# Magicyw/Quadruped-PyMPC-TAMOLS

Hardware: AMD Instinct MI355X
Metric: SRBD rollouts/sec + p50 MPC-step ms at N=10k H=12; 1/2/4/8 GPU (higher is better)
Workload: dtype f32; 1 GPU; go2_trot_flat_mppi_n10000_h12_zo; num_samples=10000, rows_per_gpu=10000, horizon=12, method=mppi, parametrization=zero_order, robot=go2, gait=trot, parallelism=single GPU

## Files before the change

### quadruped-pympc-tamols_amd/csrc/srbd_device.h

```cpp
#pragma once

#include <utility>

#include "srbd_jaxrng.h"
#include "srbd_launch.h"

namespace srbd {

#ifdef SRBD_ROLLOUT_STAMPS
constexpr int RSTAMP_N = 6, RSTAMP_BLOCKS = 8192;
__device__ uint64_t g_rstamp[RSTAMP_BLOCKS * RSTAMP_N];
#define SRBD_RSTAMP(i)                                                                  \
    do {                                                                                \
        if (threadIdx.x == 0 && blockIdx.x < RSTAMP_BLOCKS) {                           \
            asm volatile("s_waitcnt vmcnt(0) lgkmcnt(0)" ::: "memory");                 \
            g_rstamp[blockIdx.x * RSTAMP_N + (i)] = __builtin_amdgcn_s_memrealtime(); \
        }                                                                               \
    } while (0)
__device__ uint64_t g_lstamp[RSTAMP_BLOCKS * 8];
__device__ uint64_t g_fstamp[64];
#define SRBD_LSTAMP(i)                                                                            \
    do {                                                                                          \
        if (threadIdx.x == 0 && blockIdx.x < RSTAMP_BLOCKS)                                       \
            g_lstamp[blockIdx.x * 8 + (i)] = __builtin_amdgcn_s_memrealtime();                    \
// ... 182 lines not shown
    const size_t ldn = (size_t)mc.ldn;
    int j = first / n, k = first - j * n;
    const int sj = stride / n, sk = stride - sj * n;
    while (j < P) {
        const int r = mc.row0 + k;
        const float v = r > 0 ? jax_noise_value(mc, k0, k1, r, j, part) : 0.0f;
        __hip_atomic_store(&job.noise[(size_t)j * ldn + k], v, __ATOMIC_RELAXED, __HIP_MEMORY_SCOPE_AGENT);
        k += sk;
        j += sj;
        if (k >= n) {
            k -= n;
            ++j;
        }
    }
}

__device__ __forceinline__ void advance_key(const ModelConst& mc, StepInput* in, int inc) {
    const uint64_t cc = (((uint64_t)in->ctr_hi << 32) | in->ctr_lo) + (uint64_t)inc;
    in->ctr_lo = (uint32_t)cc;
    in->ctr_hi = (uint32_t)(cc >> 32);
    if (mc.rng != RNG_PHILOX) {
        const uint64_t key = jax_next_key(((uint64_t)in->seed_hi << 32) | in->seed_lo, mc.rng == RNG_JAX, inc);
        in->seed_lo = (uint32_t)key;
        in->seed_hi = (uint32_t)(key >> 32);
    }
}

__device__ __forceinline__ void rng_items(const ModelConst& mc, const StepInput* __restrict__ in, const RngJob& job,
                                          int first, int stride) {
    uint64_t seed = job.seed, ctr = job.ctr;
    if (job.dev_ctr) {
        seed = ((uint64_t)in->seed_hi << 32) | in->seed_lo;
        ctr = (((uint64_t)in->ctr_hi << 32) | in->ctr_lo) + (uint64_t)job.ctr_offset;
        if (mc.rng != RNG_PHILOX) seed = jax_next_key(seed, mc.rng == RNG_JAX, job.ctr_offset);
    }
    if (mc.rng != RNG_PHILOX) return jax_rng_items(mc, seed, job, first, stride);
    const int n = mc.n_local, nq = mc.P / 4;
    int q = first / n, k = first - q * n;
    const int sq = stride / n, sk = stride - sq * n;
    while (q < nq) {
        rng_item(mc, in->sigma, (uint32_t)seed, (uint32_t)(seed >> 32), (uint32_t)ctr, (uint32_t)(ctr >> 32), k, q,
                 job.noise);
        k += sk;
        q += sq;
        if (k >= n) {
            k -= n;
            ++q;
        }
    }
}

__host__ __device__ constexpr int chunk_index(int n, int H, int S) { return (n * S) / H; }

template <int N>
struct IntC {
    static constexpr int value = N;
};
template <class F, int... Ns>
__device__ __forceinline__ void unroll_seq(F&& f, std::integer_sequence<int, Ns...>) {
    (f(IntC<Ns>{}), ...);
}

__device__ __forceinline__ void st_rec(float* p, float v) {
    __hip_atomic_store(reinterpret_cast<uint32_t*>(p), __float_as_uint(v), __ATOMIC_RELAXED, __HIP_MEMORY_SCOPE_AGENT);
}
__device__ __forceinline__ float ld_rec(const float* p) {
    return __uint_as_float(
        __hip_atomic_load(reinterpret_cast<const uint32_t*>(p), __ATOMIC_RELAXED, __HIP_MEMORY_SCOPE_AGENT));
}
template <int U>
__device__ __forceinline__ void stage_recs16(const float* __restrict__ src, float* dst, int n) {
    const int tid = threadIdx.x, T = blockDim.x, n4 = n >> 2;
    const auto rs = __builtin_amdgcn_make_buffer_rsrc((void*)src, (short)0, n * 4, 0x00020000);
    float4* d4 = reinterpret_cast<float4*>(dst);
    for (int i0 = 0; i0 < n4; i0 += U * T) {
        float4 v[U];
#pragma unroll
        for (int u = 0; u < U; ++u) {
            const auto x = __builtin_amdgcn_raw_buffer_load_b128(rs, 16 * (i0 + u * T + tid), 0, 16);
            v[u] = make_float4(__uint_as_float(x[0]), __uint_as_float(x[1]), __uint_as_float(x[2]),
                               __uint_as_float(x[3]));
        }
#pragma unroll
        for (int u = 0; u < U; ++u) {
            const int i = i0 + u * T + tid;
            if (i < n4) d4[i] = v[u];
        }
    }
}
template <int U>
__device__ __forceinline__ void stage_recs(const float* __restrict__ src, float* dst, int n) {
    const int tid = threadIdx.x, T = blockDim.x, n2 = n >> 1;
    const uint64_t* s2 = reinterpret_cast<const uint64_t*>(src);
    uint64_t* d2 = reinterpret_cast<uint64_t*>(dst);
    for (int i0 = 0; i0 < n2; i0 += U * T) {
        uint64_t v[U];
#pragma unroll
        for (int u = 0; u < U; ++u) {
            const int i = i0 + u * T + tid;
            v[u] = i < n2 ? __hip_atomic_load(s2 + i, __ATOMIC_RELAXED, __HIP_MEMORY_SCOPE_AGENT) : 0ull;
        }
#pragma unroll
        for (int u = 0; u < U; ++u) {
            const int i = i0 + u * T + tid;
            if (i < n2) d2[i] = v[u];
        }
    }
}


__device__ __forceinline__ void fold_node_lds(const ModelConst& mc, const float* st, int rec_stride, int nb, float* G) {
    __shared__ float sc_sh[TREE_FAN];
    __shared__ float gh_sh[2];
    __shared__ uint64_t gk_sh[MAXK + 1];
    const int tid = threadIdx.x, T = blockDim.x;
    const int P = mc.P, K = mc.K;
    const bool rs = mc.method == SRBD_RANDOM_SAMPLING;
    if (tid < 64) {
        const float* R = st + (size_t)tid * rec_stride;
        const bool have = tid < nb;
        const float m = have ? R[0] : 0.0f;
        const uint32_t row = have ? __float_as_uint(R[2]) : 0u;
        const uint64_t key = have ? ((uint64_t)__float_as_uint(m) << 32) | row : KEY_NONE;
        const uint64_t gk = wave_min_u64(key);
        const float beta = __uint_as_float((uint32_t)(gk >> 32));
        if (key == gk) gh_sh[1] = R[3];
        if (tid == 0) {
            gh_sh[0] = beta;
            gk_sh[MAXK] = gk;
        }
        if (have) sc_sh[tid] = rs ? 1.0f : expf(-1.0f * (m - beta));
        if (tid == 0) gk_sh[0] = gk;
    }
    __syncthreads();
    SRBD_LSTAMP(4);
    if (!rs) {
        for (int j = tid; j <= P; j += T) {
            const int off = j < P ? REC_HDR + j : 1;
            float a = 0.0f;
            int cb = 0;
            for (; cb + 8 <= nb; cb += 8) {
                float x[8];
#pragma unroll
                for (int u = 0; u < 8; ++u) x[u] = st[(size_t)(cb + u) * rec_stride + off];
#pragma unroll
                for (int u = 0; u < 8; ++u) a = a + sc_sh[cb + u] * x[u];
            }
            for (; cb < nb; ++cb) a = a + sc_sh[cb] * st[(size_t)cb * rec_stride + off];
            st_rec(&G[off], a);
        }
    }
    SRBD_LSTAMP(5);
    if (tid == 0) {
        st_rec(&G[0], gh_sh[0]);
        if (rs) st_rec(&G[1], 1.0f);
        st_rec(&G[2], __uint_as_float((uint32_t)gk_sh[MAXK]));
        st_rec(&G[3], gh_sh[1]);
    }
    if (tid < K) {
        const uint64_t kk = gk_sh[tid];
        st_rec(&G[REC_HDR + P + 2 * tid], __uint_as_float((uint32_t)kk));
        st_rec(&G[REC_HDR + P + 2 * tid + 1], __uint_as_float((uint32_t)(kk >> 32)));
    }
}

__device__ __forceinline__ bool level1_fold(const ModelConst& mc, const float* __restrict__ recs, int rec_stride,
                                            const GroupArgs& grp, int nroll, int lpb, float* st) {
    __shared__ int last_sh;
    const int tid = threadIdx.x;
    const int bpg = TREE_FAN / lpb;
    const int g = (int)blockIdx.x / bpg;
    const int nblk = min(bpg, nroll - g * bpg);
    const int nb = min(TREE_FAN, mc.nleaf - g * TREE_FAN);
    SRBD_LSTAMP(0);
    asm volatile("s_waitcnt vmcnt(0)" ::: "memory");
    __syncthreads();
    SRBD_LSTAMP(1);
    if (tid == 0) {
        const uint32_t old = __hip_atomic_fetch_add(grp.cnt + g, 1u, __ATOMIC_RELAXED, __HIP_MEMORY_SCOPE_AGENT);
        last_sh = old == (uint32_t)(nblk - 1);
    }
    __syncthreads();
    if (!last_sh) return false;
    SRBD_LSTAMP(2);
    if (tid == 0) __hip_atomic_store(grp.cnt + g, 0u, __ATOMIC_RELAXED, __HIP_MEMORY_SCOPE_AGENT);
    stage_recs16<5>(recs + (size_t)g * TREE_FAN * rec_stride, st, nb * rec_stride);
    __syncthreads();
    SRBD_LSTAMP(3);
    fold_node_lds(mc, st, rec_stride, nb, grp.grecs + (size_t)g * rec_stride);
    return true;
}

template <int CTRL, int ROWMASK>
__device__ __forceinline__ float dpp_f32(float v) {
    return __int_as_float(__builtin_amdgcn_update_dpp(0, __float_as_int(v), CTRL, ROWMASK, 0xF, false));
}
template <int LEVELS>
__device__ __forceinline__ float lane_tree_f32(float v) {
    v = v + dpp_f32<0x111, 0xF>(v);
    v = v + dpp_f32<0x112, 0xF>(v);
    v = v + dpp_f32<0x114, 0xF>(v);
    v = v + dpp_f32<0x118, 0xF>(v);
    if constexpr (LEVELS >= 5) v = v + dpp_f32<0x142, 0xA>(v);
    if constexpr (LEVELS >= 6) v = v + dpp_f32<0x143, 0xC>(v);
    return v;
}
__device__ __forceinline__ float wave_sum_f32(float v) { return lane_tree_f32<6>(v); }

constexpr int REGEN_QUADS = 16;
template <int SPL, int RG>
__device__ __forceinline__ void leaf_wsum_lanes(const ModelConst& mc, const StepInput* __restrict__ in,
                                                const float* __restrict__ base, bool zs, const float* e_sh,
                                                float* rbuf, int rec_stride, int k0, int gen = 0) {
    constexpr int CB = SPL == 4 ? 8 : 12;
    constexpr int LPL = 64 / SPL;
    const int lane = threadIdx.x & 63, w = threadIdx.x >> 6, NW = blockDim.x >> 6;
    const int P = mc.P;
    const size_t ldn = (size_t)mc.ldn;
    float e[SPL];
#pragma unroll
    for (int u = 0; u < SPL; ++u) e[u] = e_sh[SPL * lane + u];
    float* rec = rbuf + (lane / LPL) * rec_stride;
    const bool writer = (lane % LPL) == LPL - 1;
    int jreg = 0;
    if constexpr (RG && SPL == 4) {
        if (RG == 2 || (mc.method == SRBD_MPPI && mc.rng == RNG_PHILOX && in->noise_scaled == 0 && 4 * REGEN_QUADS <= P)) {
            const uint32_t key0 = in->seed_lo, key1 = in->seed_hi, c2 = in->ctr_lo, c3 = in->ctr_hi;
            const int nq = RG == 2 ? gen - 1 : REGEN_QUADS;
            for (int q = w; q < nq; q += NW) {
                float zq[4][SPL];
#pragma unroll
                for (int u = 0; u < SPL; ++u) {
                    const int k = k0 + SPL * lane + u, r = mc.row0 + k;
                    uint32_t c[4] = {(uint32_t)(r - 1), (uint32_t)q, c2, c3};
                    philox4x32_10(c, key0, key1);
                    float v[4];
                    box_muller(c[0], c[1], v[0], v[1]);
                    box_muller(c[2], c[3], v[2], v[3]);
                    const bool live = r > 0 && k < mc.n_local;
#pragma unroll
                    for (int i = 0; i < 4; ++i) zq[i][u] = live ? mc.sigma_mppi * v[i] : 0.0f;
                }
#pragma unroll
                for (int i = 0; i < 4; ++i) {
                    float p[SPL];
#pragma unroll
                    for (int u = 0; u < SPL; ++u) p[u] = e[u] * (zq[i][u] * 1.0f);
                    float a = (p[0] + p[1]) + (p[2] + p[3]);
                    a = lane_tree_f32<4>(a);
                    if (writer) rec[REC_HDR + 4 * q + i] = a;
                }
            }
            jreg = 4 * nq;
        }
    }
    for (int j0 = jreg + w; j0 <= P; j0 += CB * NW) {
        float z[CB][SPL];
#pragma unroll
        for (int b = 0; b < CB; ++b) {
            const int j = j0 + b * NW;
            const float* col = base + (size_t)(j < P ? j : 0) * ldn + SPL * lane;
            if constexpr (SPL == 4) {
                const float4 v = *reinterpret_cast<const float4*>(col);
                z[b][0] = v.x, z[b][1] = v.y, z[b][2] = v.z, z[b][3] = v.w;
            } else {
                const float2 v = *reinterpret_cast<const float2*>(col);
                z[b][0] = v.x, z[b][1] = v.y;
            }
        }
#pragma unroll
        for (int b = 0; b < CB; ++b) {
            const int j = j0 + b * NW;
            if (j > P) break;
            float p[SPL];
            if (j < P) {
                const float sj = zs ? in->sigma[j] : 1.0f;
#pragma unroll
                for (int u = 0; u < SPL; ++u) p[u] = e[u] * (z[b][u] * sj);
            } else {
#pragma unroll
                for (int u = 0; u < SPL; ++u) p[u] = e[u];
            }
            float a;
            if constexpr (SPL == 4)
                a = (p[0] + p[1]) + (p[2] + p[3]);
            else
                a = p[0] + p[1];
            a = lane_tree_f32<SPL == 4 ? 4 : 5>(a);
            if (writer) rec[j < P ? REC_HDR + j : 1] = a;
        }
    }
}

template <bool ZS>
__device__ __forceinline__ void leaf_wsum_cols(const ModelConst& mc, const StepInput* __restrict__ in,
                                               const float* __restrict__ base, const float* zst, int zstride, bool zs,
                                               const float* e_sh, float* __restrict__ rec) {
    const int tid = threadIdx.x, T = blockDim.x, P = mc.P;
    const size_t ldn = (size_t)mc.ldn;
    if ((tid >> 6) == (T >> 6) - 1) {
        const float t = wave_sum_f32(e_sh[tid & 63]);
        if ((tid & 63) == 63) st_rec(&rec[1], t);
    }
    for (int j = tid; j < P; j += T) {
        const float sj = zs ? in->sigma[j] : 1.0f;
        float first = 0.0f, tot = 0.0f;
#pragma nounroll
        for (int h = 0; h < 2; ++h) {
            float lv[16];
            if constexpr (ZS) {
#pragma unroll
                for (int i = 0; i < 16; ++i) {
                    const int r = 32 * h + 2 * i;
                    lv[i] = e_sh[r] * (zst[r * zstride + j] * sj) + e_sh[r + 1] * (zst[(r + 1) * zstride + j] * sj);
                }
            } else {
                const float4* row = reinterpret_cast<const float4*>(base + (size_t)j * ldn) + 8 * h;
                float4 v[8];
#pragma unroll
                for (int i = 0; i < 8; ++i) v[i] = row[i];
#pragma unroll
                for (int i = 0; i < 8; ++i) {
                    const int r = 32 * h + 4 * i;
                    lv[2 * i] = e_sh[r] * (v[i].x * sj) + e_sh[r + 1] * (v[i].y * sj);
                    lv[2 * i + 1] = e_sh[r + 2] * (v[i].z * sj) + e_sh[r + 3] * (v[i].w * sj);
                }
            }
#pragma unroll
            for (int n = 8; n >= 1; n >>= 1)
#pragma unroll
                for (int i = 0; i < n; ++i) lv[i] = lv[2 * i] + lv[2 * i + 1];
            if (h == 0)
                first = lv[0];
            else
                tot = first + lv[0];
        }
        st_rec(&rec[REC_HDR + j], tot);
    }
}

template <bool CEMT, bool ZS = false, bool TF = false, int RG = 0>
__device__ __forceinline__ bool block_epilogue(const ModelConst& mc, const StepInput* __restrict__ in, const int SPB,
                                               int sib, bool valid, float cost, const float* __restrict__ noise,
                                               float* __restrict__ recs, int rec_stride, float tag,
                                               const GroupArgs& grp, int nroll, float* zst = nullptr,
                                               int zstride = 0) {
    __shared__ uint64_t ks[ZS ? 64 : 256];
    __shared__ float e_sh[ZS ? 64 : 256];
    __shared__ uint64_t lmin[4];
    __shared__ uint64_t lel[CEMT ? 4 : 1][CEMT ? MAXK : 1];
    __shared__ float rbuf[TF ? 4 * ((REC_HDR + MAXP + 2 * MAXK + 3) & ~3) : 1];
    const int tid = threadIdx.x, lane = tid & 63, w = tid >> 6;
    const int lpb = SPB >> 6;
    const int P = mc.P, K = mc.K;
    const int k0 = blockIdx.x * SPB;
    const bool rs = mc.method == SRBD_RANDOM_SAMPLING;
    const uint64_t key = (sib >= 0 && valid) ? cost_key(cost, (uint32_t)(mc.row0 + k0 + sib)) : KEY_NONE;
    if (sib >= 0) ks[sib] = key;
    __syncthreads();
    constexpr bool ONE = ZS && !CEMT;
    uint64_t m1 = KEY_NONE;
    if constexpr (ONE) {
        m1 = wave_min_u64(ks[lane]);
    } else if (w < lpb) {
        const uint64_t m = wave_min_u64(ks[64 * w + lane]);
        if (lane == 0) lmin[w] = m;
    }
    if constexpr (CEMT) {
        if (K > 1) {
            for (int i = tid; i < lpb * MAXK; i += (int)blockDim.x) lel[i / MAXK][i % MAXK] = KEY_NONE;
            __syncthreads();
            const int lps = (int)blockDim.x / SPB, part = tid & (lps - 1), s = tid / lps, b = s >> 6;
            const uint64_t mine = ks[s];
            const int span = 64 / lps, i0 = 64 * b + part * span;
            int cnt = 0;
            for (int i = 0; i < span; ++i) cnt += ks[i0 + i] < mine ? 1 : 0;
            if (lps >= 2) cnt += __builtin_amdgcn_mov_dpp(cnt, 0xB1, 0xF, 0xF, true);
            if (lps == 4) cnt += __builtin_amdgcn_mov_dpp(cnt, 0x4E, 0xF, 0xF, true);
            if (part == 0 && cnt < K) lel[b][cnt] = mine;
        }
    }
    if constexpr (!ONE) __syncthreads();
    SRBD_RSTAMP(3);
    if (!rs) {
        const uint64_t lm = ONE ? m1 : (sib >= 0 ? lmin[sib >> 6] : KEY_NONE);
        if (sib >= 0) e_sh[sib] = valid ? expf(-1.0f * (cost - u2f((uint32_t)(lm >> 32)))) : 0.0f;
        __syncthreads();
        const bool zs = CEMT && zs_scaled(mc, in);
        if (SPB == 64)
            leaf_wsum_cols<ZS>(mc, in, noise + k0, zst, zstride, zs, e_sh, recs + (size_t)blockIdx.x * rec_stride);
        else if constexpr (TF) {
            if (SPB == 128)
                leaf_wsum_lanes<2, RG>(mc, in, noise + k0, zs, e_sh, rbuf, rec_stride, k0);
            else
                leaf_wsum_lanes<4, RG>(mc, in, noise + k0, zs, e_sh, rbuf, rec_stride, k0, grp.gen);
        }
    }
    SRBD_RSTAMP(4);
    const bool via_lds = TF && SPB > 64;
    float* const grec = recs + (size_t)blockIdx.x * lpb * rec_stride;
    auto put = [&](int b, int off, float v) {
        if (via_lds)
            rbuf[b * rec_stride + off] = v;
        else
            st_rec(&grec[(size_t)b * rec_stride + off], v);
    };
    auto leafmin = [&](int b) { return ONE ? m1 : lmin[b]; };
    if (tid < lpb) {
        const uint64_t m = leafmin(tid);
        put(tid, 0, u2f((uint32_t)(m >> 32)));
        put(tid, 2, u2f((uint32_t)m));
        if (rs) put(tid, 1, 1.0f);
    }
    if (sib >= 0 && key == leafmin(sib >> 6)) put(sib >> 6, 3, tag);
    for (int i = tid; i < lpb * K; i += (int)blockDim.x) {
        const int b = i / K, q = i % K;
        uint64_t kk = leafmin(b);
        if constexpr (CEMT) kk = K > 1 ? lel[b][q] : kk;
        put(b, REC_HDR + P + 2 * q, u2f((uint32_t)kk));
        put(b, REC_HDR + P + 2 * q + 1, u2f((uint32_t)(kk >> 32)));
    }
    if (via_lds) {
        __syncthreads();
        for (int i = tid; i < lpb * rec_stride; i += (int)blockDim.x) st_rec(&grec[i], rbuf[i]);
    }
    if constexpr (!CEMT) {
        if (grp.gsize > 1) {
            if (grp.fast) return true;
            if constexpr (ZS) {
                return level1_fold(mc, recs, rec_stride, grp, nroll, lpb, zst);
            } else {
                __shared__ __attribute__((aligned(16))) float st[GROUP_LDS_FLOATS];
                return level1_fold(mc, recs, rec_stride, grp, nroll, lpb, st);
            }
        }
    }
    return false;
}

constexpr uint32_t GA_FREQ_LANE = 0x10000u;

__device__ __forceinline__ float ga_sample_freq(const ModelConst& mc, const StepInput* __restrict__ in, int k) {
    if (in->ga_explicit) return mc.ga_freq[k];
    const uint64_t seed = ((uint64_t)in->seed_hi << 32) | in->seed_lo;
    if (mc.rng != RNG_PHILOX)
        return in->ga_freqs[jax_choice_index((uint32_t)(seed >> 32), (uint32_t)seed, (uint64_t)(mc.row0 + k),
                                             (uint64_t)mc.N, (uint32_t)in->ga_nfreq, mc.rng == RNG_JAX)];
    uint32_t c[4] = {(uint32_t)(mc.row0 + k), GA_FREQ_LANE, in->ctr_lo, in->ctr_hi};
    philox4x32_10(c, (uint32_t)seed, (uint32_t)(seed >> 32));
    const uint32_t i = (uint32_t)(((uint64_t)c[0] * (uint32_t)in->ga_nfreq) >> 32);
    return in->ga_freqs[i];
}

__device__ __forceinline__ void ga_contact_masks(const StepInput* __restrict__ in, int H, float f, uint32_t mask[4]) {
    const float inc = in->ga_dt * f;
    float t[4];
#pragma unroll
    for (int l = 0; l < 4; ++l) {
        t[l] = in->ga_timing[l];
        mask[l] = 0u;
    }
    for (int n = 0; n < H; ++n)
#pragma unroll
        for (int l = 0; l < 4; ++l) {
            t[l] = t[l] >= 1.0f ? 0.0f : t[l];
            t[l] = t[l] + inc;
            mask[l] |= (t[l] < in->ga_duty ? 1u : 0u) << n;
        }
}

}
```

### quadruped-pympc-tamols_amd/csrc/srbd_kernels.hip

```cpp
#include "srbd_device.h"

#include <cstdlib>

namespace srbd {

__global__ void __launch_bounds__(256) rng_kernel(const ModelConst mc, const StepInput* __restrict__ in,
                                                  const RngJob job) {
    if (job.gate && (*job.gate & ARM_CANCEL)) return;
    rng_items(mc, in, job, blockIdx.x * 256 + threadIdx.x, gridDim.x * 256);
}

__global__ void __launch_bounds__(256) transpose_kernel(const float* __restrict__ src, int n, int P, int ldn,
                                                        float* __restrict__ dst) {
    __shared__ float tile[32][33];
    const int bx = blockIdx.x * 32, by = blockIdx.y * 32;
    const int tx = threadIdx.x & 31, ty = threadIdx.x >> 5;
    for (int i = ty; i < 32; i += 8) {
        const int row = bx + i, col = by + tx;
        tile[i][tx] = (row < n && col < P) ? src[(size_t)row * P + col] : 0.0f;
    }
    __syncthreads();
    for (int i = ty; i < 32; i += 8) {
        const int col = by + i, row = bx + tx;
        if (col < P && row < n) dst[(size_t)col * ldn + row] = tile[tx][i];
// ... 31 lines not shown
};
__device__ __forceinline__ QuadLane quad_lane(const ModelConst& mc, int c) {
    QuadLane L;
    L.c = c;
    L.g = c == 2 ? -9.81f : 0.0f;
    L.Ir0 = sel3(c, mc.inertia[0], mc.inertia[3], mc.inertia[6]);
    L.Ir1 = sel3(c, mc.inertia[1], mc.inertia[4], mc.inertia[7]);
    L.Ir2 = sel3(c, mc.inertia[2], mc.inertia[5], mc.inertia[8]);
    L.Ii0 = sel3(c, mc.Iinv[0], mc.Iinv[3], mc.Iinv[6]);
    L.Ii1 = sel3(c, mc.Iinv[1], mc.Iinv[4], mc.Iinv[7]);
    L.Ii2 = sel3(c, mc.Iinv[2], mc.Iinv[5], mc.Iinv[8]);
    return L;
}

struct QuadRB {
    float er, R0, R1, R2, a1;
};
__device__ __forceinline__ QuadRB quad_rb_prep(const QuadLane& L, float r, float w) {
    const int c = L.c;
    float sn, cs;
    sincos_(r, &sn, &cs);
    const float sr = qp<QP_B0>(sn), cr = qp<QP_B0>(cs);
    const float sp = qp<QP_B1>(sn), cp = qp<QP_B1>(cs);
    const float sy = qp<QP_B2>(sn), cy = qp<QP_B2>(cs);
    const float w0 = qp<QP_B0>(w), w1 = qp<QP_B1>(w), w2 = qp<QP_B2>(w);
    float k1, k2;
    euler_rate_coefs(c, sr, cr, sp, cp, k1, k2);
    const float kw1 = k1 * w1;
    const float er0 = w0 + kw1;
    const float er = (c == 0 ? er0 : kw1) + k2 * w2;
    const float A = c == 1 ? sr : cr;
    const float B0 = c == 1 ? -cr : sr, B1 = c == 1 ? cr : -sr;
    const float Asp = A * sp;
    const float r0a = cp * cy, r0b = Asp * cy + B0 * sy;
    const float r1a = cp * sy, r1b = Asp * sy + B1 * cy;
    const float r2b = A * cp;
    const float R0 = c == 0 ? r0a : r0b;
    const float R1 = c == 0 ? r1a : r1b;
    const float R2 = c == 0 ? -sp : r2b;
    const float Iw = L.Ir0 * w0 + L.Ir1 * w1 + L.Ir2 * w2;
    const float wx = (-qp<QP_NEXT2>(w)) * qp<QP_NEXT>(Iw) + qp<QP_NEXT>(w) * qp<QP_NEXT2>(Iw);
    const float a1 = L.Ii0 * qp<QP_B0>(wx) + L.Ii1 * qp<QP_B1>(wx) + L.Ii2 * qp<QP_B2>(wx);
    return QuadRB{er, R0, R1, R2, a1};
}
__device__ __forceinline__ void quad_rb_apply(const ModelConst& mc, const QuadLane& L, const QuadRB& q, float temp,
                                              float temp2, float dt, float& p, float& v, float& r, float& w) {
    const float lin = mc.inv_m * temp + L.g;
    const float Rt = q.R0 * qp<QP_B0>(temp2) + q.R1 * qp<QP_B1>(temp2) + q.R2 * qp<QP_B2>(temp2);
    const float a2 = L.Ii0 * qp<QP_B0>(Rt) + L.Ii1 * qp<QP_B1>(Rt) + L.Ii2 * qp<QP_B2>(Rt);
    const float aa = -q.a1 + a2;
    const float pn = p + v * dt, vn = v + lin * dt, rn = r + q.er * dt, wn = w + aa * dt;
    p = pn;
    v = vn;
    r = rn;
    w = wn;
}
__device__ __forceinline__ void quad_rb_apply3(const ModelConst& mc, const QuadLane& L, const QuadRB& q, float temp,
                                               float t2x, float t2y, float t2z, float dt, float& p, float& v, float& r,
                                               float& w) {
    const float lin = mc.inv_m * temp + L.g;
    const float Rt = q.R0 * t2x + q.R1 * t2y + q.R2 * t2z;
    const float a2 = L.Ii0 * qp<QP_B0>(Rt) + L.Ii1 * qp<QP_B1>(Rt) + L.Ii2 * qp<QP_B2>(Rt);
    const float aa = -q.a1 + a2;
    const float pn = p + v * dt, vn = v + lin * dt, rn = r + q.er * dt, wn = w + aa * dt;
    p = pn;
    v = vn;
    r = rn;
    w = wn;
}
__device__ __forceinline__ void quad_rigid_body(const ModelConst& mc, const QuadLane& L, float temp, float temp2,
                                                float dt, float& p, float& v, float& r, float& w) {
    quad_rb_apply(mc, L, quad_rb_prep(L, r, w), temp, temp2, dt, p, v, r, w);
}

__device__ __forceinline__ float quad_cross(float vl, float fl) {
    const float vn1 = qp<QP_NEXT>(vl), vn2 = qp<QP_NEXT2>(vl);
    const float fn1 = qp<QP_NEXT>(fl), fn2 = qp<QP_NEXT2>(fl);
    return (-vn2) * fn1 + vn1 * fn2;
}

template <int NT, bool XG>
__device__ void final_merge(const ModelConst& mc, const StepInput* in, const float* noise, int rec_stride,
                            const GroupArgs& grp, float* lds);
__device__ void fast_tail(const ModelConst& mc, const StepInput* in, const float* noise, const float* recs,
                          int rec_stride, const GroupArgs& grp, int nroll, float* st);

#ifndef SRBD_QUAD_WPE
#define SRBD_QUAD_WPE 4
#endif
template <int KIND, int HT, int ST, bool CEMT, bool EXT, int FM = 0, bool KS = false, bool GEN = false>
__global__ void __launch_bounds__(512) __attribute__((amdgpu_waves_per_eu(SRBD_QUAD_WPE))) rollout_quad_kernel(
                                                           const std::conditional_t<KS, StepInputK, KsNone> ksi,
                                                           const ModelConst mc, const StepInput* __restrict__ in_dev,
                                                           const float* __restrict__ noise, float* __restrict__ costs,
                                                           float* __restrict__ recs, int rec_stride,
    const RngJob next_rng, int nroll, const GroupArgs grp) {
    const StepInput* __restrict__ in;
    if constexpr (KS) {
        (void)ksi;
        const auto ka = (const __attribute__((address_space(4))) StepInput*)__builtin_amdgcn_kernarg_segment_ptr();
        in = (const StepInput*)ka;
        if (blockIdx.x == 0) {
            const auto src = (const __attribute__((address_space(4))) uint32_t*)ka;
            uint32_t* dst = reinterpret_cast<uint32_t*>(const_cast<StepInput*>(in_dev));
            for (int i = threadIdx.x; i < (int)(sizeof(StepInputK) / 4); i += blockDim.x) dst[i] = src[i];
        }
    } else {
        in = in_dev;
    }
    if (grp.gate && (*grp.gate & ARM_CANCEL)) {
        if (FM && blockIdx.x == 0 && threadIdx.x == 0)
            __hip_atomic_store(grp.flag, grp.seq | ARM_CANCEL, __ATOMIC_RELAXED, __HIP_MEMORY_SCOPE_SYSTEM);
        return;
    }
    SRBD_RSTAMP(0);
#if SRBD_PRIO
    if ((int)blockIdx.x < nroll && nroll >= SRBD_PRIO_MIN) __builtin_amdgcn_s_setprio(SRBD_PRIO);
#endif
    if ((int)blockIdx.x >= nroll) {
        rng_items(mc, in, next_rng, ((int)blockIdx.x - nroll) * (int)blockDim.x + (int)threadIdx.x,
                  ((int)gridDim.x - nroll) * (int)blockDim.x);
        SRBD_RSTAMP(5);
        return;
    }

    constexpr bool CT = HT > 0 && (KIND == SRBD_ZERO_ORDER || ST > 0);
    const int SPB = (int)blockDim.x >> 2;
    const int H = CT ? HT : mc.H;
    const int S = CT ? ST : mc.S;
    const int PL = CT ? (KIND == SRBD_ZERO_ORDER ? 3 * HT : (KIND == SRBD_LINEAR_SPLINE ? 3 * (ST + 1) : 12 * ST))
                      : mc.PL;
    constexpr bool ZST = CT && KIND == SRBD_ZERO_ORDER && !EXT && HT <= 12;
    static_assert(!GEN || (ZST && HT % 4 == 0 && !CEMT), "GEN: the zero-order LDS-staged form, H % 4 == 0");
    constexpr int PCT = ZST ? 12 * HT : 1;
    constexpr int ZSTR = PCT + 1;
    __shared__ __attribute__((aligned(16))) float zst[ZST ? (64 * ZSTR > GROUP_LDS_FLOATS ? 64 * ZSTR : GROUP_LDS_FLOATS) : 1];
    __shared__ float bls[ZST ? PCT : 1];
    __shared__ float sls[ZST && CEMT ? PCT : 1];
    const int tid = threadIdx.x;
    const int q4 = tid & 3;
    const int c = q4 < 3 ? q4 : 2;
    const int sib = tid >> 2;
    const int k = blockIdx.x * SPB + sib;
    const bool valid = k < mc.n_local;
    const size_t ldn = (size_t)mc.ldn;
    const float* __restrict__ nz = noise + k;
    const float* __restrict__ best = in->best;
    const bool zs = CEMT && zs_scaled(mc, in);

    const QuadLane L = quad_lane(mc, c);
    const float Qp = sel3(c, mc.Q[0], mc.Q[1], mc.Q[2]), Qv = sel3(c, mc.Q[3], mc.Q[4], mc.Q[5]);
    const float Qr = sel3(c, mc.Q[6], mc.Q[7], mc.Q[8]), Qw = sel3(c, mc.Q[9], mc.Q[10], mc.Q[11]);
    const float* st = in->state;
    const float* rf = in->ref;
    const float rp = sel3(c, rf[0], rf[1], rf[2]), rv = sel3(c, rf[3], rf[4], rf[5]);
    const float rr = sel3(c, rf[6], rf[7], rf[8]), rw = sel3(c, rf[9], rf[10], rf[11]);
    float feet[4];
#pragma unroll
    for (int l = 0; l < 4; ++l) feet[l] = sel3(c, st[12 + 3 * l], st[13 + 3 * l], st[14 + 3 * l]);
    float p = sel3(c, st[0], st[1], st[2]), v = sel3(c, st[3], st[4], st[5]);
    float r = sel3(c, st[6], st[7], st[8]), w = sel3(c, st[9], st[10], st[11]);
    float cost = 0.0f;
    const float rwc = sel3(c, mc.cost_r[0], mc.cost_r[1], mc.cost_r[2]);
    float fprev[4];
    constexpr bool LEGP = !EXT;
    const int lq = q4;
    uint32_t lmask[4];
#pragma unroll
    for (int l = 0; l < 4; ++l) lmask[l] = lq == l ? ~0u : 0u;
    float footL[3];
#pragma unroll
    for (int q = 0; q < 3; ++q) footL[q] = st[12 + 3 * lq + q];
    constexpr int NCL = ZST ? HT : 1;
    float clreg[NCL];
    if constexpr (ZST) {
#pragma unroll
        for (int n = 0; n < HT; ++n) clreg[n] = in->contact[lq][n];
    }

    constexpr int NPRE = !CT ? 1 : (KIND == SRBD_ZERO_ORDER ? HT : (KIND == SRBD_LINEAR_SPLINE ? ST + 1 : 4 * ST));
    float pre[LEGP ? 3 : 4][NPRE];
    const int cblk = LEGP ? lq * PL
                          : (KIND == SRBD_ZERO_ORDER ? c * HT : (KIND == SRBD_LINEAR_SPLINE ? c * (ST + 1) : 4 * c));
    const auto nrs = __builtin_amdgcn_make_buffer_rsrc((void*)noise, (short)0, mc.P * mc.ldn * 4, 0x00020000);
    const int voff = (cblk * mc.ldn + k) * 4;
    const float* __restrict__ bl = best + cblk;
    const float* __restrict__ sl = in->sigma + cblk;
    if constexpr (ZST) {
        for (int j = tid; j < PCT; j += 256) {
            bls[j] = best[j];
            if constexpr (CEMT) sls[j] = in->sigma[j];
        }
    }
    auto load_slot = [&](const int i) __attribute__((always_inline)) {
#pragma unroll
        for (int l = 0; l < (LEGP ? 3 : 4); ++l) {
            const int jr = LEGP ? (KIND == SRBD_ZERO_ORDER ? l * HT + i
                                   : (KIND == SRBD_LINEAR_SPLINE ? l * (ST + 1) + i : 10 * (i >> 2) + 4 * l + (i & 3)))
                                : l * PL + (KIND == SRBD_CUBIC_SPLINE ? 10 * (i >> 2) + (i & 3) : i);
#ifdef SRBD_DIAG_NOLOAD
            const float nzv = (float)(voff + jr * mc.ldn) * 1e-9f;
#else
            const float nzv = __uint_as_float(__builtin_amdgcn_raw_buffer_load_b32(nrs, voff, jr * mc.ldn * 4, 0));
#endif
            if constexpr (ZST) {
                pre[l][i] = nzv;
            } else if constexpr (CEMT) {
                const float sj = sl[jr];
                pre[l][i] = bl[jr] + nzv * (zs ? sj : 1.0f);
            } else {
                pre[l][i] = bl[jr] + nzv;
            }
        }
    };
    constexpr int PW = (EXT && KIND == SRBD_ZERO_ORDER) ? (NPRE < 4 ? NPRE : 4) : NPRE;
    constexpr int CLEAD = 2;
    constexpr bool CWIN = CT && CEMT && KIND == SRBD_CUBIC_SPLINE && ST > 1;
    if constexpr (GEN) {
    } else if constexpr (CWIN) {
#pragma unroll
        for (int i = 0; i < 4; ++i) load_slot(i);
    } else if constexpr (CT) {
#pragma unroll
        for (int i = 0; i < PW; ++i) load_slot(i);
    }
    if constexpr (ZST) {
        asm volatile("s_waitcnt lgkmcnt(0)" ::: "memory");
        __builtin_amdgcn_s_barrier();
    }

    float dep = p;
    auto gen4 = [&](const int s, auto is) __attribute__((always_inline)) {
        const int r = mc.row0 + k;
        const bool live = r > 0 && valid;
        const uint32_t d = (uint32_t)(r - 1);
#pragma unroll
        for (int q = 0; q < 3; ++q) {
            uint32_t cc[4] = {d, (uint32_t)(lq * (PL / 4) + q * (HT / 4) + s), is->ctr_lo, is->ctr_hi};
            philox4x32_10(cc, is->seed_lo, is->seed_hi);
            float v[4];
            box_muller(cc[0], cc[1], v[0], v[1]);
            box_muller(cc[2], cc[3], v[2], v[3]);
#pragma unroll
            for (int i = 0; i < 4; ++i) pre[q][(4 * s + i) % NPRE] = live ? mc.sigma_mppi * v[i] : 0.0f;
        }
    };
    auto step = [&](const int n, auto EX) __attribute__((always_inline)) {
        if constexpr (GEN)
            if (n % 4 == 0) gen4(n / 4, step_ptr(in, cost));
        if constexpr (CT && PW < NPRE)
            if (n + PW < NPRE) load_slot(n + PW);
        if constexpr (CWIN) {
#pragma unroll
            for (int q = 1; q < (CWIN ? ST : 1); ++q) {
                const int at = q * HT / ST - CLEAD;
                if (n == (at > 0 ? at : 0))
#pragma unroll
                    for (int i = 4 * q; i < 4 * q + 4; ++i) load_slot(i);
            }
        }
        const auto is = step_ptr(in, dep);
        float cl[4] = {0.0f, 0.0f, 0.0f, 0.0f};
        if constexpr (!ZST)
#pragma unroll
            for (int l = 0; l < 4; ++l) cl[l] = is->contact[l][n];
        const float fref = is->fzref[n];
        const float dt = mc.dts[n];
        const float sq = mc.sq[n], somq = mc.somq[n], sa = mc.sa[n], sb = mc.sb[n], scc = mc.sc[n], sd = mc.sd[n];
        const int idx = CT && KIND != SRBD_ZERO_ORDER ? chunk_index(n, HT, ST) : mc.sidx[n];
        float temp, temp2, ex = 0.0f;
        if constexpr (LEGP) {
            const float clq = ZST ? clreg[ZST ? n : 0]
                                  : __uint_as_float((__float_as_uint(cl[0]) & lmask[0]) | (__float_as_uint(cl[1]) & lmask[1]) |
                                                    (__float_as_uint(cl[2]) & lmask[2]) | (__float_as_uint(cl[3]) & lmask[3]));
            const int lbase = lq * PL;
            auto PQ = [&](int q, int i, int j) {
                if constexpr (ZST) {
                    if constexpr (CEMT) return bls[lbase + j] + pre[q][i] * (zs ? sls[lbase + j] : 1.0f);
                    return bls[lbase + j] + pre[q][i];
                } else if constexpr (CT) {
                    return pre[q][i];
                } else {
                    const float z = nz[(size_t)(lbase + j) * ldn];
                    return best[lbase + j] + (zs ? z * in->sigma[lbase + j] : z);
                }
            };
            float rq[3];
#pragma unroll
            for (int q = 0; q < 3; ++q) {
                if (KIND == SRBD_ZERO_ORDER) {
                    rq[q] = PQ(q, n, n + q * H);
                } else if (KIND == SRBD_LINEAR_SPLINE) {
                    const int o = idx + q * (S + 1);
                    rq[q] = somq * PQ(q, idx, o) + sq * PQ(q, idx + 1, o + 1);
                } else {
                    const int o = 10 * idx + 4 * q;
                    const float p0 = PQ(q, 4 * idx, o), p1 = PQ(q, 4 * idx + 1, o + 1), p2 = PQ(q, 4 * idx + 2, o + 2),
                                p3 = PQ(q, 4 * idx + 3, o + 3);
                    const float phi = 0.5f * ((p2 - p1) + (p1 - p0));
                    const float phin = 0.5f * ((p3 - p2) + (p2 - p1));
                    rq[q] = sa * p1 + sb * phi + scc * p2 + sd * phin;
                }
            }
            const float fz = clamp_cs((fref + rq[2]) * clq, mc.grf_min, mc.grf_max);
            const float lo = mc.neg_mu * fz, hi = mc.mu * fz;
            const float fx = clamp_cs(third(rq[0] * clq), lo, hi), fy = clamp_cs(third(rq[1] * clq), lo, hi);
            const float vx = footL[0] - qp<QP_B0>(p), vy = footL[1] - qp<QP_B1>(p), vz = footL[2] - qp<QP_B2>(p);
            float sm[6] = {fx * clq, fy * clq, fz * clq, ((-vz) * fy + vy * fz) * clq, (vz * fx + (-vx) * fz) * clq,
                           ((-vy) * fx + vx * fy) * clq};
#pragma unroll
            for (int i = 0; i < 6; ++i) {
                sm[i] = sm[i] + qp<QP_XOR1>(sm[i]);
                sm[i] = sm[i] + qp<QP_XOR2>(sm[i]);
            }
            temp = sel3(c, sm[0], sm[1], sm[2]);
            temp2 = sel3(c, sm[3], sm[4], sm[5]);
            dep = sm[5];
            quad_rb_apply3(mc, L, quad_rb_prep(L, r, w), temp, sm[3], sm[4], sm[5], dt, p, v, r, w);
        } else {
        float tf[4], tt[4];
#pragma unroll
        for (int l = 0; l < 4; ++l) {
            const int base = l * PL;
            auto P = [&](int i, int j) {
                if constexpr (CT) {
                    return pre[l][i];
                } else {
                    const float z = nz[(size_t)(base + j) * ldn];
                    return best[base + j] + (zs ? z * in->sigma[base + j] : z);
                }
            };
            float raw;
            if (KIND == SRBD_ZERO_ORDER) {
                raw = P(n, n + c * H);
            } else if (KIND == SRBD_LINEAR_SPLINE) {
                const int o = idx + c * (S + 1);
                raw = somq * P(idx, o) + sq * P(idx + 1, o + 1);
            } else {
                const int o = 10 * idx + 4 * c;
                const float p0 = P(4 * idx, o), p1 = P(4 * idx + 1, o + 1), p2 = P(4 * idx + 2, o + 2),
                            p3 = P(4 * idx + 3, o + 3);
                const float phi = 0.5f * ((p2 - p1) + (p1 - p0));
                const float phin = 0.5f * ((p3 - p2) + (p2 - p1));
                raw = sa * p1 + sb * phi + scc * p2 + sd * phin;
            }
            float zp = clamp_cs((fref + raw) * cl[l], mc.grf_min, mc.grf_max);
            const float xy = third(raw * cl[l]);
            const float fz = qp<QP_B2>(c == 2 ? zp : xy);
            const float f = c == 2 ? fz : clamp_cs(xy, mc.neg_mu * fz, mc.mu * fz);
            tf[l] = f * cl[l];
            tt[l] = quad_cross(feet[l] - p, f) * cl[l];
            if constexpr (decltype(EX)::value) {
                const float u = c == 2 ? f - (cl[l] != 0.0f ? fref : 0.0f) : f;
                float term = (u * rwc) * u;
                if (n > 0) {
                    const float d = f - fprev[l];
                    term = term + (d * mc.cost_smooth) * d;
                }
                {
                    float vv = fabsf(xy) - mc.mu * fz;
                    vv = vv > 0.0f ? vv : 0.0f;
                    const float cone = (vv * mc.cost_cone) * vv;
                    term = c < 2 ? term + cone : term;
                }
                ex = ex + term;
                fprev[l] = f;
            }
        }
        temp = (tf[0] + tf[1]) + (tf[2] + tf[3]);
        temp2 = (tt[0] + tt[1]) + (tt[2] + tt[3]);
        dep = temp2;
        quad_rigid_body(mc, L, temp, temp2, dt, p, v, r, w);
        }
        const float ep = p - rp, ev = v - rv, er_ = r - rr, ew = w - rw;
        const float tp = (ep * Qp) * ep, tv = (ev * Qv) * ev, tr = (er_ * Qr) * er_, tw = (ew * Qw) * ew;
        cost = cost + (((tp + tv) + tr) + tw);
        if constexpr (decltype(EX)::value) {
            cost = cost + ex;
            asm volatile("" : "+v"(cost));
        }
    };
    auto horizon = [&](auto EX) __attribute__((always_inline)) {
        if constexpr (CT) {
            unroll_seq([&](auto nc) { step(decltype(nc)::value, EX); },
                       std::make_integer_sequence<int, (CT ? HT : 1)>{});
        } else {
            for (int n = 0; n < H; ++n) step(n, EX);
        }
    };
    horizon(std::bool_constant<EXT>{});
    SRBD_RSTAMP(2);
    cost = (qp<QP_B0>(cost) + qp<QP_B1>(cost)) + qp<QP_B2>(cost);
    cost = cost + in->cost_feet;
    if (isnan(cost) || isinf(cost)) cost = 1000000.0f;
    if (valid && q4 == 0 && costs) costs[k] = cost;
    if constexpr (ZST) {
#pragma unroll
        for (int q = 0; q < 3; ++q)
#pragma unroll
            for (int i = 0; i < NPRE; ++i) zst[sib * ZSTR + lq * PL + q * HT + i] = pre[q][i];
    }
#ifdef SRBD_DIAG_NOEPI
    if (tid == 0) recs[blockIdx.x] = cost;
    return;
#endif
    const bool glast = block_epilogue<CEMT, ZST>(mc, in, SPB, q4 == 0 ? sib : -1, valid, cost, noise, recs, rec_stride,
                                                 0.0f, grp, nroll, ZST ? zst : nullptr, ZSTR);
    if constexpr (FM && ZST && !CEMT) {
        if (FM == 1 && grp.fast) {
            if (glast) fast_tail(mc, in, noise, recs, rec_stride, grp, nroll, zst);
        } else if (glast) {
            final_merge<256, FM == 2>(mc, in, noise, rec_stride, grp, zst);
        }
    }
    SRBD_RSTAMP(5);
}

template <int KIND, int HT>
__global__ void __launch_bounds__(512) rollout_ga_quad_kernel(const ModelConst mc, const StepInput* __restrict__ in,
                                                              const float* __restrict__ noise,
                                                              float* __restrict__ costs, float* __restrict__ recs,
                                                              int rec_stride, const RngJob next_rng, int nroll, const GroupArgs grp) {
    if (grp.gate && (*grp.gate & ARM_CANCEL)) return;
    if ((int)blockIdx.x >= nroll) {
        rng_items(mc, in, next_rng, ((int)blockIdx.x - nroll) * (int)blockDim.x + (int)threadIdx.x,
                  ((int)gridDim.x - nroll) * (int)blockDim.x);
        return;
    }
    const int H = HT > 0 ? HT : mc.H, S = mc.S, PL = mc.PL;
    const int tid = threadIdx.x;
    const int q4 = tid & 3;
    const int c = q4 < 3 ? q4 : 2;
    const int sib = tid >> 2;
    const int SPB = (int)blockDim.x >> 2;
    const int k = blockIdx.x * SPB + sib;
    const bool valid = k < mc.n_local;
    const size_t ldn = (size_t)mc.ldn;
    const float* __restrict__ nz = noise + k;
    const float* __restrict__ best = in->best;

    const float f = ga_sample_freq(mc, in, k);
    uint32_t mask[4];
    ga_contact_masks(in, H, f, mask);
    float seg[4];
#pragma unroll
    for (int l = 0; l < 4; ++l) seg[l] = ((float)__popc(mask[l]) + 1.0f) / (float)S;
    int cnt[4] = {-1, -1, -1, -1};

    const QuadLane L = quad_lane(mc, c);
    const float Qp = sel3(c, mc.Q[0], mc.Q[1], mc.Q[2]), Qv = sel3(c, mc.Q[3], mc.Q[4], mc.Q[5]);
    const float Qr = sel3(c, mc.Q[6], mc.Q[7], mc.Q[8]), Qw = sel3(c, mc.Q[9], mc.Q[10], mc.Q[11]);
    const float* st_ = in->state;
    const float* rf = in->ref;
    const float rp = sel3(c, rf[0], rf[1], rf[2]), rv = sel3(c, rf[3], rf[4], rf[5]);
    const float rr = sel3(c, rf[6], rf[7], rf[8]), rw = sel3(c, rf[9], rf[10], rf[11]);
    float feet[4];
#pragma unroll
    for (int l = 0; l < 4; ++l) feet[l] = sel3(c, st_[12 + 3 * l], st_[13 + 3 * l], st_[14 + 3 * l]);
    float p = sel3(c, st_[0], st_[1], st_[2]), v = sel3(c, st_[3], st_[4], st_[5]);
    float r = sel3(c, st_[6], st_[7], st_[8]), w = sel3(c, st_[9], st_[10], st_[11]);
    float cost = 0.0f;
    constexpr int UNR = HT > 0 ? HT : 1;
#pragma unroll UNR
    for (int n = 0; n < H; ++n) {
        float cl[4];
#pragma unroll
        for (int l = 0; l < 4; ++l) {
            const uint32_t b = (mask[l] >> n) & 1u;
            cl[l] = b ? 1.0f : 0.0f;
            cnt[l] += (int)b;
        }
        const float ns = ((cl[0] + cl[1]) + cl[2]) + cl[3];
        const float fref = mc.fz_ns[(int)ns];
        float tf[4], tt[4];
#pragma unroll
        for (int l = 0; l < 4; ++l) {
            const int base = l * PL;
            auto acc = [&](int j) {
                j = j < 0 ? j + PL : j;
                return best[base + j] + nz[(size_t)(base + j) * ldn];
            };
            const int stc = cnt[l];
            float raw;
            if (KIND == SRBD_ZERO_ORDER) {
                raw = acc(stc + c * H);
            } else {
                int idx = 0;
                for (int i = 0; i <= S; ++i)
                    if (stc >= in->ga_cb[i]) idx = i;
                float tau = (float)stc / seg[l];
                tau = tau - (float)idx;
                const float q = tau / 1.0f;
                if (KIND == SRBD_LINEAR_SPLINE) {
                    const float omq = 1.0f - q;
                    const int o = idx + c * (S + 1);
                    raw = omq * acc(o) + q * acc(o + 1);
                } else {
                    const float a = 2.0f * q * q * q - 3.0f * q * q + 1.0f;
                    const float bb = (q * q * q - 2.0f * q * q + q) * 1.0f;
                    const float cc = -2.0f * q * q * q + 3.0f * q * q;
                    const float d = (q * q * q - q * q) * 1.0f;
                    const int o = 10 * idx + 4 * c;
                    const float p0 = acc(o), p1 = acc(o + 1), p2 = acc(o + 2), p3 = acc(o + 3);
                    const float phi = 0.5f * ((p2 - p1) + (p1 - p0));
                    const float phin = 0.5f * ((p3 - p2) + (p2 - p1));
                    raw = a * p1 + bb * phi + cc * p2 + d * phin;
                }
            }
            const float zp = clamp_cs((fref + raw) * cl[l], mc.grf_min, mc.grf_max);
            const float xy = third(raw * cl[l]);
            const float fz = qp<QP_B2>(c == 2 ? zp : xy);
            const float fo = c == 2 ? fz : clamp_cs(xy, mc.neg_mu * fz, mc.mu * fz);
            tf[l] = fo * cl[l];
            tt[l] = quad_cross(feet[l] - p, fo) * cl[l];
        }
        const float temp = (tf[0] + tf[1]) + (tf[2] + tf[3]), temp2 = (tt[0] + tt[1]) + (tt[2] + tt[3]);
        quad_rigid_body(mc, L, temp, temp2, mc.dts[n], p, v, r, w);
        const float ep = p - rp, ev = v - rv, er_ = r - rr, ew = w - rw;
        const float tp = (ep * Qp) * ep, tv = (ev * Qv) * ev, tr = (er_ * Qr) * er_, tw = (ew * Qw) * ew;
        cost = cost + (((tp + tv) + tr) + tw);
    }
    cost = (qp<QP_B0>(cost) + qp<QP_B1>(cost)) + qp<QP_B2>(cost);
    cost = cost + in->cost_feet;
    const float df = f - 1.3f;
    cost = cost + (df * 100.0f) * df;
    if (isnan(cost) || isinf(cost)) cost = 1000000.0f;
    if (valid && q4 == 0 && costs) costs[k] = cost;
    block_epilogue<false>(mc, in, SPB, q4 == 0 ? sib : -1, valid, cost, noise, recs, rec_stride, f, grp, nroll);
}

__device__ __forceinline__ uint64_t rec_key(const float* R, int P, int q) {
    return ((uint64_t)f2u(R[REC_HDR + P + 2 * q + 1]) << 32) | (uint64_t)f2u(R[REC_HDR + P + 2 * q]);
}

constexpr int MERGE_THREADS = 1024;
constexpr int MERGE_RPT = 8;
constexpr int MERGE_STAGE_THREADS = 512;
template <int NT>
struct TopkLds {
    static constexpr int NCT = (NT / 64) * MAXK + MAXK > MAXK * MAXK ? (NT / 64) * MAXK + MAXK : MAXK * MAXK;
    uint64_t keys[NT > MAXK * MAXK ? NT : MAXK * MAXK];
    uint64_t cand[NCT];
    int cand_r[NCT];
    int cnt[MAXK * MAXK];
    uint64_t top[MAXK], ntop[MAXK];
    int top_r[MAXK], ntop_r[MAXK];
    int sel[MAXK];
};
template <int NT>
__device__ __forceinline__ void block_topk_rank(const float* __restrict__ recs, int nrec, int rec_stride, int P, int K,
                                                uint64_t* elite, TopkLds<NT>& t) {
    constexpr int NW = NT / 64;
    const int tid = threadIdx.x, T = NT, wv = tid >> 6;
    const int NC = NW * K + K;
    if (tid < K) {
        t.top[tid] = KEY_NONE;
        t.top_r[tid] = 0;
    }
    for (int base = 0; base < nrec; base += T) {
        const int r = base + tid;
        const uint64_t x = r < nrec ? rec_key(recs + (size_t)r * rec_stride, P, 0) : KEY_NONE;
        t.keys[tid] = x;
        for (int i = tid; i < NW * K; i += T) t.cand[i] = KEY_NONE;
        __syncthreads();
        const uint64_t* wk = t.keys + (wv << 6);
        int cnt = 0;
#pragma unroll 16
        for (int j = 0; j < 64; ++j) cnt += wk[j] < x ? 1 : 0;
        if (cnt < K && x != KEY_NONE) {
            t.cand[wv * K + cnt] = x;
            t.cand_r[wv * K + cnt] = r;
        }
        if (tid < K) {
            t.cand[NW * K + tid] = t.top[tid];
            t.cand_r[NW * K + tid] = t.top_r[tid];
            t.ntop[tid] = KEY_NONE;
        }
        __syncthreads();
        if (tid < NC) {
            const uint64_t y = t.cand[tid];
            int c2 = 0;
            for (int j = 0; j < NC; ++j) c2 += t.cand[j] < y ? 1 : 0;
            if (c2 < K && y != KEY_NONE) {
                t.ntop[c2] = y;
                t.ntop_r[c2] = t.cand_r[tid];
            }
        }
        __syncthreads();
        if (tid < K) {
            t.top[tid] = t.ntop[tid];
            t.top_r[tid] = t.ntop_r[tid];
        }
        __syncthreads();
    }
    const int KK = K * K;
    for (int i = tid; i < KK; i += T) {
        const int e = i / K, q = i - e * K;
        t.keys[i] = t.top[e] != KEY_NONE ? rec_key(recs + (size_t)t.top_r[e] * rec_stride, P, q) : KEY_NONE;
    }
    if (tid < K) elite[tid] = KEY_NONE;
    __syncthreads();
    for (int i = tid; i < KK; i += T) {
        const uint64_t y = t.keys[i];
        int c3 = 0;
        for (int j = 0; j < KK; ++j) c3 += t.keys[j] < y ? 1 : 0;
        if (c3 < K && y != KEY_NONE) elite[c3] = y;
    }
}

template <int NT>
__device__ __forceinline__ void block_topk_nodes(const float* __restrict__ recs, int nrec, int rec_stride, int P,
                                                 int K, const uint64_t* nk, uint64_t* elite, TopkLds<NT>& t,
                                                 uint64_t* dbg = nullptr) {
    const int tid = threadIdx.x, KK = K * K;
#define TOPK_MARK(i) \
    if (dbg && tid == 0 && blockIdx.x < 2) dbg[32 * blockIdx.x + 25 + (i)] = __builtin_amdgcn_s_memrealtime()
    const int n1 = (nrec + TREE_FAN - 1) / TREE_FAN;
    if (tid < n1) {
        const uint64_t y = nk[tid];
        int c = 0;
#pragma unroll 8
        for (int g = 0; g < n1; ++g) c += nk[g] < y ? 1 : 0;
        if (c < K && y != KEY_NONE) t.sel[c] = tid;
    }
    __syncthreads();
    TOPK_MARK(0);
    for (int i = tid; i < K * TREE_FAN; i += NT) {
        const int sl = i / TREE_FAN, g = t.sel[sl];
        if (g < 0) continue;
        const uint64_t* nodek = t.keys + g * TREE_FAN;
        const uint64_t y = nodek[i % TREE_FAN];
        if (y == KEY_NONE) continue;
        int c = 0;
#pragma unroll
        for (int j = 0; j < TREE_FAN; ++j) c += nodek[j] < y ? 1 : 0;
        if (c < K) {
            t.cand[sl * K + c] = y;
            t.cand_r[sl * K + c] = g * TREE_FAN + i % TREE_FAN;
        }
    }
    __syncthreads();
    static_assert(MAXK <= 31, "binary lifting from a step of 16");
    auto table_ranks = [&](const uint64_t* tab) {
        for (int i = tid; i < KK * K; i += NT) {
            const int c = i / K, b = i - c * K;
            const uint64_t y = tab[c];
            if (y == KEY_NONE) continue;
            const uint64_t* row = tab + b * K;
            int n = 0;
#pragma unroll
            for (int s = 16; s >= 1; s >>= 1)
                if (n + s <= K && row[n + s - 1] < y) n += s;
            if (n) atomicAdd(&t.cnt[c], n);
        }
    };
    TOPK_MARK(1);
    table_ranks(t.cand);
    __syncthreads();
    TOPK_MARK(2);
    for (int c = tid; c < KK; c += NT) {
        const uint64_t y = t.cand[c];
        const int n = t.cnt[c];
        if (y != KEY_NONE && n < K) {
            t.top[n] = y;
            t.top_r[n] = t.cand_r[c];
        }
    }
    __syncthreads();
    for (int i = tid; i < KK; i += NT) {
        const int e = i / K, q = i - e * K;
        t.keys[i] = t.top[e] != KEY_NONE ? rec_key(recs + (size_t)t.top_r[e] * rec_stride, P, q) : KEY_NONE;
        t.cnt[i] = 0;
    }
    if (tid < K) elite[tid] = KEY_NONE;
    __syncthreads();
    TOPK_MARK(3);
    table_ranks(t.keys);
    __syncthreads();
    TOPK_MARK(4);
#undef TOPK_MARK
    for (int i = tid; i < KK; i += NT) {
        const uint64_t y = t.keys[i];
        const int n = t.cnt[i];
        if (y != KEY_NONE && n < K) elite[n] = y;
    }
}

template <int NT>
struct alignas(16) MergeShared {
    uint64_t red[NT / 64];
    uint64_t elite[MAXK];
    int elite_src[MAXK];
    TopkLds<NT> tk;
    float Vs[MAXP + 1];
    float nb[MAXP];
    float tag_sh;
    float tail_sh[4][40];
    float osh[sizeof(StepOutput) / sizeof(float)];
};
template <class IN>
__device__ __forceinline__ void merge_tail_load(const IN* in, int qc, float* tail_pre) {
    tail_pre[0] = in->fzref[0];
#pragma unroll
    for (int l = 0; l < 4; ++l) tail_pre[1 + l] = in->contact[l][0];
// ... 1352 lines not shown
```

Measured before the change: 450.3 million rollouts/s.

## Split ZS weighted-sum across 8-lane groups with DPP reduction; stream zst stores per step

The shared-memory weighted column sum for the zero-order stash path now assigns each column to an 8-lane group. Each lane holds 8 cached weights, loads several columns per batch, and reduces with DPP row shifts instead of one thread summing 64 rows serially. The rollout kernel also writes its per-step noise stash to shared memory inside the horizon loop instead of after it, which shortens register live ranges. The risks are less column parallelism per thread, extra shared stores inside the hot loop, and reliance on the stride layout (PZ = zstride-1).

Measured after the change: 433.2 million rollouts/s. 0.962x the previous value.

```diff
diff --git a/quadruped-pympc-tamols_amd/csrc/srbd_device.h b/quadruped-pympc-tamols_amd/csrc/srbd_device.h
--- a/quadruped-pympc-tamols_amd/csrc/srbd_device.h
+++ b/quadruped-pympc-tamols_amd/csrc/srbd_device.h
@@ -508,29 +508,55 @@
         const float t = wave_sum_f32(e_sh[tid & 63]);
         if ((tid & 63) == 63) st_rec(&rec[1], t);
     }
+    if constexpr (ZS) {
+        constexpr int CPR = 32, NB = 5;
+        const int PZ = zstride - 1;
+        const int ch = tid & 7, jj = tid >> 3;
+        float e[8];
+#pragma unroll
+        for (int u = 0; u < 8; ++u) e[u] = e_sh[8 * ch + u];
+        const float* zrow = zst + 8 * ch * zstride;
+        for (int jb = jj; jb - jj < PZ; jb += NB * CPR) {
+            float z[NB][8], sj[NB];
+#pragma unroll
+            for (int b = 0; b < NB; ++b) {
+                if (jb - jj + b * CPR >= PZ) break;
+                const int j = jb + b * CPR, jc = j < PZ ? j : 0;
+#pragma unroll
+                for (int u = 0; u < 8; ++u) z[b][u] = zrow[u * zstride + jc];
+                sj[b] = zs ? in->sigma[jc] : 1.0f;
+            }
+#pragma unroll
+            for (int b = 0; b < NB; ++b) {
+                if (jb - jj + b * CPR >= PZ) break;
+                const int j = jb + b * CPR;
+                float p[8];
+#pragma unroll
+                for (int u = 0; u < 8; ++u) p[u] = e[u] * (z[b][u] * sj[b]);
+                float a = ((p[0] + p[1]) + (p[2] + p[3])) + ((p[4] + p[5]) + (p[6] + p[7]));
+                a = a + dpp_f32<0x111, 0xF>(a);
+                a = a + dpp_f32<0x112, 0xF>(a);
+                a = a + dpp_f32<0x114, 0xF>(a);
+                if (ch == 7 && j < PZ) st_rec(&rec[REC_HDR + j], a);
+            }
+        }
+        return;
+    }
     for (int j = tid; j < P; j += T) {
         const float sj = zs ? in->sigma[j] : 1.0f;
         float first = 0.0f, tot = 0.0f;
 #pragma nounroll
         for (int h = 0; h < 2; ++h) {
             float lv[16];
-            if constexpr (ZS) {
-#pragma unroll
-                for (int i = 0; i < 16; ++i) {
-                    const int r = 32 * h + 2 * i;
-                    lv[i] = e_sh[r] * (zst[r * zstride + j] * sj) + e_sh[r + 1] * (zst[(r + 1) * zstride + j] * sj);
-                }
-            } else {
-                const float4* row = reinterpret_cast<const float4*>(base + (size_t)j * ldn) + 8 * h;
-                float4 v[8];
-#pragma unroll
-                for (int i = 0; i < 8; ++i) v[i] = row[i];
-#pragma unroll
-                for (int i = 0; i < 8; ++i) {
-                    const int r = 32 * h + 4 * i;
-                    lv[2 * i] = e_sh[r] * (v[i].x * sj) + e_sh[r + 1] * (v[i].y * sj);
-                    lv[2 * i + 1] = e_sh[r + 2] * (v[i].z * sj) + e_sh[r + 3] * (v[i].w * sj);
-                }
+            const float4* row = reinterpret_cast<const float4*>(base + (size_t)j * ldn) + 8 * h;
+            float4 v[8];
+#pragma unroll
+            for (int i = 0; i < 8; ++i) v[i] = row[i];
+#pragma unroll
+            for (int i = 0; i < 8; ++i) {
+                const int r = 32 * h + 4 * i;
+                lv[2 * i] = e_sh[r] * (v[i].x * sj) + e_sh[r + 1] * (v[i].y * sj);
+                lv[2 * i + 1] = e_sh[r + 2] * (v[i].z * sj) + e_sh[r + 3] * (v[i].w * sj);
             }
 #pragma unroll
             for (int n = 8; n >= 1; n >>= 1)
diff --git a/quadruped-pympc-tamols_amd/csrc/srbd_kernels.hip b/quadruped-pympc-tamols_amd/csrc/srbd_kernels.hip
--- a/quadruped-pympc-tamols_amd/csrc/srbd_kernels.hip
+++ b/quadruped-pympc-tamols_amd/csrc/srbd_kernels.hip
@@ -357,6 +357,10 @@
                     rq[q] = sa * p1 + sb * phi + scc * p2 + sd * phin;
                 }
             }
+            if constexpr (ZST) {
+#pragma unroll
+                for (int q = 0; q < 3; ++q) zst[sib * ZSTR + lq * PL + q * HT + n] = pre[q][n];
+            }
             const float fz = clamp_cs((fref + rq[2]) * clq, mc.grf_min, mc.grf_max);
             const float lo = mc.neg_mu * fz, hi = mc.mu * fz;
             const float fx = clamp_cs(third(rq[0] * clq), lo, hi), fy = clamp_cs(third(rq[1] * clq), lo, hi);
@@ -449,12 +453,6 @@
     cost = cost + in->cost_feet;
     if (isnan(cost) || isinf(cost)) cost = 1000000.0f;
     if (valid && q4 == 0 && costs) costs[k] = cost;
-    if constexpr (ZST) {
-#pragma unroll
-        for (int q = 0; q < 3; ++q)
-#pragma unroll
-            for (int i = 0; i < NPRE; ++i) zst[sib * ZSTR + lq * PL + q * HT + i] = pre[q][i];
-    }
 #ifdef SRBD_DIAG_NOEPI
     if (tid == 0) recs[blockIdx.x] = cost;
     return;
```
